# NTT123/vietTTS

Hardware: NVIDIA H100
Metric: audio_samples_per_sec (higher is better)
Workload: dtype f32 (bf16x3 split products on wgmma tensor cores, fp32 accumulate/storage)

## Files before the change

viettts_b200/csrc/tc_common.cuh:

```cuda
#pragma once
#include <cuda_bf16.h>
#include <stdint.h>

namespace tcx {

constexpr long long SPIN_TIMEOUT = 4000000000LL;

__device__ __forceinline__ uint32_t smem_u32(const void* p) { return (uint32_t)__cvta_generic_to_shared(p); }

__device__ __forceinline__ void mbar_init(uint64_t* bar, uint32_t count) {
  asm volatile("mbarrier.init.shared::cta.b64 [%0], %1;" ::"r"(smem_u32(bar)), "r"(count));
}
__device__ __forceinline__ void mbar_arrive(uint64_t* bar) {
  asm volatile("mbarrier.arrive.shared::cta.b64 _, [%0];" ::"r"(smem_u32(bar)) : "memory");
}
__device__ __forceinline__ void mbar_expect_tx(uint64_t* bar, uint32_t bytes) {
  asm volatile("mbarrier.arrive.expect_tx.shared::cta.b64 _, [%0], %1;" ::"r"(smem_u32(bar)), "r"(bytes) : "memory");
}
__device__ __forceinline__ bool mbar_try_wait(uint64_t* bar, uint32_t parity) {
  uint32_t ok;
  asm volatile(
      "{\n\t.reg .pred p;\n\t"
      "mbarrier.try_wait.parity.shared::cta.b64 p, [%1], %2;\n\t"
      "selp.u32 %0, 1, 0, p;\n\t}"
// ... 44 lines not shown
  if constexpr (F16) TCX_WGMMA_N32("f16"); else TCX_WGMMA_N32("bf16");
}
#define TCX_WGMMA_N64(TY)  \
  asm volatile(  \
      "{\n\t.reg .pred p;\n\t"  \
      "setp.ne.b32 p, %34, 0;\n\t"  \
      "wgmma.mma_async.sync.aligned.m64n64k16.f32." TY "." TY " "  \
      "{%0, %1, %2, %3, %4, %5, %6, %7, %8, %9, %10, %11, %12, %13, %14, %15, %16, %17, %18, %19, %20, %21, %22, %23, %24, %25, %26, %27, %28, %29, %30, %31}, "  \
      "%32, %33, p, 1, 1, 0, 0;\n\t}"  \
      : "+f"(d[0]), "+f"(d[1]), "+f"(d[2]), "+f"(d[3]), "+f"(d[4]), "+f"(d[5]), "+f"(d[6]), "+f"(d[7]), "+f"(d[8]), "+f"(d[9]), "+f"(d[10]), "+f"(d[11]), "+f"(d[12]), "+f"(d[13]), "+f"(d[14]), "+f"(d[15]), "+f"(d[16]), "+f"(d[17]), "+f"(d[18]), "+f"(d[19]), "+f"(d[20]), "+f"(d[21]), "+f"(d[22]), "+f"(d[23]), "+f"(d[24]), "+f"(d[25]), "+f"(d[26]), "+f"(d[27]), "+f"(d[28]), "+f"(d[29]), "+f"(d[30]), "+f"(d[31])  \
      : "l"(adesc), "l"(bdesc), "r"(accumulate)  \
  )
template <bool F16>
__device__ __forceinline__ void wgmma_n64(float (&d)[32], uint64_t adesc, uint64_t bdesc, uint32_t accumulate) {
  if constexpr (F16) TCX_WGMMA_N64("f16"); else TCX_WGMMA_N64("bf16");
}
#define TCX_WGMMA_N128(TY)  \
  asm volatile(  \
      "{\n\t.reg .pred p;\n\t"  \
      "setp.ne.b32 p, %66, 0;\n\t"  \
      "wgmma.mma_async.sync.aligned.m64n128k16.f32." TY "." TY " "  \
      "{%0, %1, %2, %3, %4, %5, %6, %7, %8, %9, %10, %11, %12, %13, %14, %15, %16, %17, %18, %19, %20, %21, %22, %23, %24, %25, %26, %27, %28, %29, %30, %31, %32, %33, %34, %35, %36, %37, %38, %39, %40, %41, %42, %43, %44, %45, %46, %47, %48, %49, %50, %51, %52, %53, %54, %55, %56, %57, %58, %59, %60, %61, %62, %63}, "  \
      "%64, %65, p, 1, 1, 0, 0;\n\t}"  \
      : "+f"(d[0]), "+f"(d[1]), "+f"(d[2]), "+f"(d[3]), "+f"(d[4]), "+f"(d[5]), "+f"(d[6]), "+f"(d[7]), "+f"(d[8]), "+f"(d[9]), "+f"(d[10]), "+f"(d[11]), "+f"(d[12]), "+f"(d[13]), "+f"(d[14]), "+f"(d[15]), "+f"(d[16]), "+f"(d[17]), "+f"(d[18]), "+f"(d[19]), "+f"(d[20]), "+f"(d[21]), "+f"(d[22]), "+f"(d[23]), "+f"(d[24]), "+f"(d[25]), "+f"(d[26]), "+f"(d[27]), "+f"(d[28]), "+f"(d[29]), "+f"(d[30]), "+f"(d[31]), "+f"(d[32]), "+f"(d[33]), "+f"(d[34]), "+f"(d[35]), "+f"(d[36]), "+f"(d[37]), "+f"(d[38]), "+f"(d[39]), "+f"(d[40]), "+f"(d[41]), "+f"(d[42]), "+f"(d[43]), "+f"(d[44]), "+f"(d[45]), "+f"(d[46]), "+f"(d[47]), "+f"(d[48]), "+f"(d[49]), "+f"(d[50]), "+f"(d[51]), "+f"(d[52]), "+f"(d[53]), "+f"(d[54]), "+f"(d[55]), "+f"(d[56]), "+f"(d[57]), "+f"(d[58]), "+f"(d[59]), "+f"(d[60]), "+f"(d[61]), "+f"(d[62]), "+f"(d[63])  \
      : "l"(adesc), "l"(bdesc), "r"(accumulate)  \
  )
template <bool F16>
__device__ __forceinline__ void wgmma_n128(float (&d)[64], uint64_t adesc, uint64_t bdesc, uint32_t accumulate) {
  if constexpr (F16) TCX_WGMMA_N128("f16"); else TCX_WGMMA_N128("bf16");
}
#define TCX_WGMMA_N256(TY)  \
  asm volatile(  \
      "{\n\t.reg .pred p;\n\t"  \
      "setp.ne.b32 p, %130, 0;\n\t"  \
      "wgmma.mma_async.sync.aligned.m64n256k16.f32." TY "." TY " "  \
      "{%0, %1, %2, %3, %4, %5, %6, %7, %8, %9, %10, %11, %12, %13, %14, %15, %16, %17, %18, %19, %20, %21, %22, %23, %24, %25, %26, %27, %28, %29, %30, %31, %32, %33, %34, %35, %36, %37, %38, %39, %40, %41, %42, %43, %44, %45, %46, %47, %48, %49, %50, %51, %52, %53, %54, %55, %56, %57, %58, %59, %60, %61, %62, %63, %64, %65, %66, %67, %68, %69, %70, %71, %72, %73, %74, %75, %76, %77, %78, %79, %80, %81, %82, %83, %84, %85, %86, %87, %88, %89, %90, %91, %92, %93, %94, %95, %96, %97, %98, %99, %100, %101, %102, %103, %104, %105, %106, %107, %108, %109, %110, %111, %112, %113, %114, %115, %116, %117, %118, %119, %120, %121, %122, %123, %124, %125, %126, %127}, "  \
      "%128, %129, p, 1, 1, 0, 0;\n\t}"  \
      : "+f"(d[0]), "+f"(d[1]), "+f"(d[2]), "+f"(d[3]), "+f"(d[4]), "+f"(d[5]), "+f"(d[6]), "+f"(d[7]), "+f"(d[8]), "+f"(d[9]), "+f"(d[10]), "+f"(d[11]), "+f"(d[12]), "+f"(d[13]), "+f"(d[14]), "+f"(d[15]), "+f"(d[16]), "+f"(d[17]), "+f"(d[18]), "+f"(d[19]), "+f"(d[20]), "+f"(d[21]), "+f"(d[22]), "+f"(d[23]), "+f"(d[24]), "+f"(d[25]), "+f"(d[26]), "+f"(d[27]), "+f"(d[28]), "+f"(d[29]), "+f"(d[30]), "+f"(d[31]), "+f"(d[32]), "+f"(d[33]), "+f"(d[34]), "+f"(d[35]), "+f"(d[36]), "+f"(d[37]), "+f"(d[38]), "+f"(d[39]), "+f"(d[40]), "+f"(d[41]), "+f"(d[42]), "+f"(d[43]), "+f"(d[44]), "+f"(d[45]), "+f"(d[46]), "+f"(d[47]), "+f"(d[48]), "+f"(d[49]), "+f"(d[50]), "+f"(d[51]), "+f"(d[52]), "+f"(d[53]), "+f"(d[54]), "+f"(d[55]), "+f"(d[56]), "+f"(d[57]), "+f"(d[58]), "+f"(d[59]), "+f"(d[60]), "+f"(d[61]), "+f"(d[62]), "+f"(d[63]), "+f"(d[64]), "+f"(d[65]), "+f"(d[66]), "+f"(d[67]), "+f"(d[68]), "+f"(d[69]), "+f"(d[70]), "+f"(d[71]), "+f"(d[72]), "+f"(d[73]), "+f"(d[74]), "+f"(d[75]), "+f"(d[76]), "+f"(d[77]), "+f"(d[78]), "+f"(d[79]), "+f"(d[80]), "+f"(d[81]), "+f"(d[82]), "+f"(d[83]), "+f"(d[84]), "+f"(d[85]), "+f"(d[86]), "+f"(d[87]), "+f"(d[88]), "+f"(d[89]), "+f"(d[90]), "+f"(d[91]), "+f"(d[92]), "+f"(d[93]), "+f"(d[94]), "+f"(d[95]), "+f"(d[96]), "+f"(d[97]), "+f"(d[98]), "+f"(d[99]), "+f"(d[100]), "+f"(d[101]), "+f"(d[102]), "+f"(d[103]), "+f"(d[104]), "+f"(d[105]), "+f"(d[106]), "+f"(d[107]), "+f"(d[108]), "+f"(d[109]), "+f"(d[110]), "+f"(d[111]), "+f"(d[112]), "+f"(d[113]), "+f"(d[114]), "+f"(d[115]), "+f"(d[116]), "+f"(d[117]), "+f"(d[118]), "+f"(d[119]), "+f"(d[120]), "+f"(d[121]), "+f"(d[122]), "+f"(d[123]), "+f"(d[124]), "+f"(d[125]), "+f"(d[126]), "+f"(d[127])  \
      : "l"(adesc), "l"(bdesc), "r"(accumulate)  \
  )
template <bool F16>
__device__ __forceinline__ void wgmma_n256(float (&d)[128], uint64_t adesc, uint64_t bdesc, uint32_t accumulate) {
  if constexpr (F16) TCX_WGMMA_N256("f16"); else TCX_WGMMA_N256("bf16");
}

template <int N, bool F16 = false>
__device__ __forceinline__ void wgmma(float (&d)[N / 2], uint64_t adesc, uint64_t bdesc, uint32_t accumulate) {
  if constexpr (N == 32) wgmma_n32<F16>(d, adesc, bdesc, accumulate);
  else if constexpr (N == 64) wgmma_n64<F16>(d, adesc, bdesc, accumulate);
  else if constexpr (N == 128) wgmma_n128<F16>(d, adesc, bdesc, accumulate);
  else wgmma_n256<F16>(d, adesc, bdesc, accumulate);
}

__device__ __forceinline__ void wgmma_rs_n32(float (&d)[16], const uint32_t (&a)[4], uint64_t bdesc, uint32_t accumulate) {
  asm volatile(
      "{\n\t.reg .pred p;\n\t"
      "setp.ne.b32 p, %21, 0;\n\t"
      "wgmma.mma_async.sync.aligned.m64n32k16.f32.bf16.bf16 "
      "{%0, %1, %2, %3, %4, %5, %6, %7, %8, %9, %10, %11, %12, %13, %14, %15}, "
      "{%16, %17, %18, %19}, %20, p, 1, 1, 0;\n\t}"
      : "+f"(d[0]), "+f"(d[1]), "+f"(d[2]), "+f"(d[3]), "+f"(d[4]), "+f"(d[5]), "+f"(d[6]), "+f"(d[7]), "+f"(d[8]), "+f"(d[9]), "+f"(d[10]), "+f"(d[11]), "+f"(d[12]), "+f"(d[13]), "+f"(d[14]), "+f"(d[15])
      : "r"(a[0]), "r"(a[1]), "r"(a[2]), "r"(a[3]), "l"(bdesc), "r"(accumulate));
}
__device__ __forceinline__ void wgmma_rs_n64(float (&d)[32], const uint32_t (&a)[4], uint64_t bdesc, uint32_t accumulate) {
  asm volatile(
      "{\n\t.reg .pred p;\n\t"
      "setp.ne.b32 p, %37, 0;\n\t"
      "wgmma.mma_async.sync.aligned.m64n64k16.f32.bf16.bf16 "
      "{%0, %1, %2, %3, %4, %5, %6, %7, %8, %9, %10, %11, %12, %13, %14, %15, %16, %17, %18, %19, %20, %21, %22, %23, %24, %25, %26, %27, %28, %29, %30, %31}, "
      "{%32, %33, %34, %35}, %36, p, 1, 1, 0;\n\t}"
      : "+f"(d[0]), "+f"(d[1]), "+f"(d[2]), "+f"(d[3]), "+f"(d[4]), "+f"(d[5]), "+f"(d[6]), "+f"(d[7]), "+f"(d[8]), "+f"(d[9]), "+f"(d[10]), "+f"(d[11]), "+f"(d[12]), "+f"(d[13]), "+f"(d[14]), "+f"(d[15]), "+f"(d[16]), "+f"(d[17]), "+f"(d[18]), "+f"(d[19]), "+f"(d[20]), "+f"(d[21]), "+f"(d[22]), "+f"(d[23]), "+f"(d[24]), "+f"(d[25]), "+f"(d[26]), "+f"(d[27]), "+f"(d[28]), "+f"(d[29]), "+f"(d[30]), "+f"(d[31])
      : "r"(a[0]), "r"(a[1]), "r"(a[2]), "r"(a[3]), "l"(bdesc), "r"(accumulate));
}

template <int N>
__device__ __forceinline__ void wgmma_rs(float (&d)[N / 2], const uint32_t (&a)[4], uint64_t bdesc, uint32_t accumulate) {
  if constexpr (N == 32) wgmma_rs_n32(d, a, bdesc, accumulate);
  else wgmma_rs_n64(d, a, bdesc, accumulate);
}
__device__ __forceinline__ void ldmatrix_x4(uint32_t (&r)[4], uint32_t saddr) {
  asm volatile("ldmatrix.sync.aligned.m8n8.x4.shared.b16 {%0, %1, %2, %3}, [%4];"
               : "=r"(r[0]), "=r"(r[1]), "=r"(r[2]), "=r"(r[3]) : "r"(saddr) : "memory");
}

__device__ __forceinline__ void named_bar(int id, int nthreads) { asm volatile("bar.sync %0, %1;" ::"r"(id), "r"(nthreads) : "memory"); }

__device__ __forceinline__ float4 ldg_pf256(const float* p) {
  float4 v;
  asm volatile("ld.global.nc.L2::256B.v4.f32 {%0, %1, %2, %3}, [%4];" : "=f"(v.x), "=f"(v.y), "=f"(v.z), "=f"(v.w) : "l"(p));
  return v;
}

__device__ __forceinline__ float lrelu(float v, float s) { return fmaxf(v, s * v); }

__device__ __forceinline__ void split4(const float4 v, uint2& hi, uint2& lo) {
  const __nv_bfloat162 h01 = __floats2bfloat162_rn(v.x, v.y);
  const __nv_bfloat162 h23 = __floats2bfloat162_rn(v.z, v.w);
  const uint32_t u01 = *reinterpret_cast<const uint32_t*>(&h01);
  const uint32_t u23 = *reinterpret_cast<const uint32_t*>(&h23);
  const float r0 = v.x - __uint_as_float(u01 << 16);
  const float r1 = v.y - __uint_as_float(u01 & 0xffff0000u);
  const float r2 = v.z - __uint_as_float(u23 << 16);
  const float r3 = v.w - __uint_as_float(u23 & 0xffff0000u);
  const __nv_bfloat162 l01 = __floats2bfloat162_rn(r0, r1);
  const __nv_bfloat162 l23 = __floats2bfloat162_rn(r2, r3);
  hi.x = u01;
  hi.y = u23;
  lo.x = *reinterpret_cast<const uint32_t*>(&l01);
  lo.y = *reinterpret_cast<const uint32_t*>(&l23);
}

__device__ __forceinline__ uint32_t f16x2_sat(float v0, float v1) {
  uint32_t r;
  asm("cvt.rn.satfinite.f16x2.f32 %0, %1, %2;" : "=r"(r) : "f"(v1), "f"(v0));
  return r;
}
__device__ __forceinline__ uint2 f16x4_sat(const float4 v) { return make_uint2(f16x2_sat(v.x, v.y), f16x2_sat(v.z, v.w)); }

}
```

viettts_b200/csrc/tc_conv.cu:

```cuda
#include <cuda_bf16.h>

#include <algorithm>

#include "tc_common.cuh"
#include "vtts_internal.cuh"

namespace {

using namespace tcx;

constexpr int NCWG = 2;
constexpr int NCONS = NCWG * 128;
constexpr int PROD_WARP = NCONS / 32;
constexpr int NCONV = 96;
constexpr int NTHREADS = NCONS + 32 + NCONV;
constexpr int NA = 4;
constexpr int HALO = 64;
constexpr int PAIR_OVERLAP = 16;
constexpr int NQ = 2;
constexpr int NREADERS = (NCONS + NCONV) / 32;

constexpr int SUB_CG = 4;
constexpr int SUB_HALO = 1;
constexpr int SUB_RS = NCWG * 64 + SUB_HALO;
// ... 218 lines not shown
          wgmma_rs<N>(acc[mt], fa_hi[mt], b_lo, 1u);
          wgmma_rs<N>(acc[mt], fa_lo[mt], b_hi, 1u);
        }
        wgmma_commit();
        wgmma_wait<0>();
        if (lane == 0) mbar_arrive(&w_empty[rw.s]);
        rw.next<NW>();
        continue;
      }
      wgmma_fence();
#pragma unroll
      for (int mt = 0; mt < MW; ++mt) {
        const uint32_t row = a_base + ((wg * MW + mt) * 64 + j * dil) * 16;
        const uint64_t a_hi = a_tmpl | (uint64_t)(row >> 4);
        const uint64_t a_lo = a_tmpl | (uint64_t)((row + 2 * RA * 16) >> 4);
        if constexpr (F16) {
          wgmma<N, true>(acc[mt], a_hi, b_hi, first);
        } else {
          wgmma<N>(acc[mt], a_hi, b_hi, first);
          wgmma<N>(acc[mt], a_hi, b_lo, 1u);
          wgmma<N>(acc[mt], a_lo, b_hi, 1u);
        }
      }
      wgmma_commit();
      wgmma_wait<1>();
      if (lane0) {
        if (pend_w >= 0) mbar_arrive(&w_empty[pend_w]);
        if (pend_a >= 0) mbar_arrive(&a_empty[pend_a]);
      }
      pend_w = (int)rw.s;
      pend_a = (A_FROM_RING && j == k - 1) ? (int)ra.s : -1;
      rw.next<NW>();
    }
    if constexpr (A_FROM_RING) ra.next<NA>();
  }
  wgmma_wait<0>();
  if (lane0) {
    if (pend_w >= 0) mbar_arrive(&w_empty[pend_w]);
    if (pend_a >= 0) mbar_arrive(&a_empty[pend_a]);
  }
}

template <int N, int NW, int NAS, bool F16>
__device__ __forceinline__ void consume_rows(float (&acc)[N / 2], int wg, uint32_t a_st_u32, uint64_t* a_full, uint64_t* a_empty, Ring& ra,
                                             uint32_t w_st_u32, uint64_t* w_full, uint64_t* w_empty, Ring& rw, int nch, int k, int dil,
                                             int* err, long long& w_a, long long& w_w) {
  const uint64_t a_tmpl = make_desc(0, SUB_RS * 16, 128);
  const uint64_t b_tmpl = make_desc(0, (F16 ? 1 : 2) * N * 16, 128);
  const bool lane0 = (threadIdx.x & 31) == 0;
  int pend_w = -1, pend_a = -1;
  for (int c0 = 0; c0 < nch; c0 += SUB_CG) {
    mbar_wait_t(&a_full[ra.s], ra.p, err, 2, w_a);
    const uint32_t a_blk = a_st_u32 + ra.s * SUB_STAGE + wg * 64 * 16;
    for (int cl = 0; cl < SUB_CG; ++cl) {
      for (int j = 0; j < k; ++j) {
        mbar_wait_t(&w_full[rw.s], rw.p, err, 3, w_w);
        const uint32_t w_base = w_st_u32 + rw.s * (N * 64);
        const uint64_t b_hi = b_tmpl | (uint64_t)(w_base >> 4);
        const uint64_t b_lo = b_tmpl | (uint64_t)((w_base + N * 16) >> 4);
        const uint32_t first = ((c0 + cl) | j) != 0 ? 1u : 0u;
        const uint32_t row = a_blk + cl * SUB_CSB + j * dil * 16;
        const uint64_t a_hi = a_tmpl | (uint64_t)(row >> 4);
        const uint64_t a_lo = a_tmpl | (uint64_t)((row + 2 * SUB_RS * 16) >> 4);
        wgmma_fence();
        if constexpr (F16) {
          wgmma<N, true>(acc, a_hi, b_hi, first);
        } else {
          wgmma<N>(acc, a_hi, b_hi, first);
          wgmma<N>(acc, a_hi, b_lo, 1u);
          wgmma<N>(acc, a_lo, b_hi, 1u);
        }
        wgmma_commit();
        wgmma_wait<1>();
        if (lane0) {
          if (pend_w >= 0) mbar_arrive(&w_empty[pend_w]);
          if (pend_a >= 0) mbar_arrive(&a_empty[pend_a]);
        }
        pend_w = (int)rw.s;
        pend_a = (cl == SUB_CG - 1 && j == k - 1) ? (int)ra.s : -1;
        rw.next<NW>();
      }
    }
    ra.next<NAS>();
  }
  wgmma_wait<0>();
  if (lane0) {
    if (pend_w >= 0) mbar_arrive(&w_empty[pend_w]);
    if (pend_a >= 0) mbar_arrive(&a_empty[pend_a]);
  }
}

__device__ __forceinline__ void cp_async16(void* smem_dst, const void* gsrc) {
  asm volatile("cp.async.cg.shared.global [%0], [%1], 16;" ::"r"(smem_u32(smem_dst)), "l"(gsrc) : "memory");
}
__device__ __forceinline__ void cp_async_commit() { asm volatile("cp.async.commit_group;" ::: "memory"); }
__device__ __forceinline__ void cp_async_wait_all() { asm volatile("cp.async.wait_all;" ::: "memory"); }

__device__ __forceinline__ void init_barriers(uint64_t* bars, int nw) {
  uint64_t* a_full = bars;
  uint64_t* a_empty = bars + NA;
  uint64_t* w_full = bars + 2 * NA;
  uint64_t* w_empty = bars + 2 * NA + nw;
  uint64_t* q_full = bars + 2 * NA + 2 * nw;
  uint64_t* q_empty = q_full + NQ;
  for (int i = 0; i < NA; ++i) { mbar_init(&a_full[i], NCONV); mbar_init(&a_empty[i], NCONS / 32); }
  for (int i = 0; i < nw; ++i) { mbar_init(&w_full[i], 1); mbar_init(&w_empty[i], NCONS / 32); }
  for (int i = 0; i < NQ; ++i) { mbar_init(&q_full[i], 1); mbar_init(&q_empty[i], NREADERS); }
  asm volatile("fence.mbarrier_init.release.cluster;" ::: "memory");
}

__device__ __forceinline__ TileQueue tile_queue(uint64_t* bars, int nw) {
  uint64_t* q_full = bars + 2 * NA + 2 * nw;
  return TileQueue{reinterpret_cast<int*>(q_full + 2 * NQ), q_full, q_full + NQ, Ring{}};
}

__device__ __forceinline__ int sub_elem(const TcLaunch& L, const TcProb& P, int tau, int col) {
  return (tau * P.out_stride + P.out_off) * L.out_ld + P.out_e0 + col;
}

#define PRODUCER_TILES                                                                     \
  TileQueue q = tile_queue(bars, NW);                                                      \
  long long w_q = 0;                                                                       \
  int t_next = blockIdx.x;                                                                 \
  q.put(t_next, L.err, w_q);                                                               \
  auto next_tile = [&]() {                                                                 \
    const int t = t_next;                                                                  \
    if (t >= 0) { t_next = take_ticket(L.sched, L.ntiles); q.put(t_next, L.err, w_q); }    \
    return t;                                                                              \
  };
#define READER_TILES                                                                       \
  TileQueue q = tile_queue(bars, NW);                                                      \
  long long w_q = 0;                                                                       \
  auto next_tile = [&]() { return q.get(L.err, w_q); };

template <int N, int EPI, int MW, bool F16, bool SUB>
__global__ void __launch_bounds__(NTHREADS, 1) tc_conv_kernel(const __grid_constant__ TcLaunch L) {
  static_assert(!SUB || EPI == 0, "sub-row output uses the plain epilogue");
  using Cfg = TcCfg<N, MW, 0, EPI == 0, SUB>;
  constexpr int R = Cfg::R, RA = Cfg::RA, NW = Cfg::NW, NAS = Cfg::NAS;
  extern __shared__ uint8_t smem_raw[];
  uint8_t* smem = (uint8_t*)(((uintptr_t)smem_raw + 1023) & ~(uintptr_t)1023);
  uint8_t* a_st = smem;
  uint8_t* w_st = smem + Cfg::A_BYTES;
  float* epi_st = reinterpret_cast<float*>(smem_raw + (w_st + NW * Cfg::W_STAGE - smem_raw));
  uint64_t* bars = reinterpret_cast<uint64_t*>(w_st + NW * Cfg::W_STAGE + Cfg::EPI_STAGE);
  uint64_t* a_full = bars;
  uint64_t* a_empty = bars + NA;
  uint64_t* w_full = bars + 2 * NA;
  uint64_t* w_empty = bars + 2 * NA + NW;

  const int tid = threadIdx.x;
  const int warp = __shfl_sync(0xffffffffu, tid >> 5, 0);
  if (tid == 0) init_barriers(bars, NW);
  __syncthreads();

  const int nch = L.Cin / 16;

  constexpr bool ROW_BOUNDS = EPI == 0;
#define TILE_LOOP_BEGIN                                                           \
  for (int tile; (tile = next_tile()) >= 0;) {                                    \
    const Tile td = decode_tile(tile, L.nprob, L.tiles_per_row);                   \
    const int b = td.b;                                                            \
    const int tau0 = td.tt * R;                                                    \
    const TcProb& P = L.p[td.pi];                                                  \
    int valid = L.T_rows, in_lo = 0, out_hi = 0;                                  \
    if (ROW_BOUNDS && P.rb) {                                                     \
// ... 110 lines not shown
#pragma unroll
        for (int mt = 0; mt < MW; ++mt) {
          const int blk = blk_row(mt);
          if (SUB ? sub_elem(L, P, blk, 0) >= e_lim : !row_ok(blk)) break;
#pragma unroll
          for (int nh = 0; nh < N / EPI_NC; ++nh) {
            if (mt + nh > 0 && P.resid) {
              fetch_pass(mt, nh);
              wait_pass();
            }
#pragma unroll
            for (int jn = 0; jn < EPI_NC / 8; ++jn) {
              const int col = jn * 8 + fc, e = (nh * (EPI_NC / 8) + jn) * 4;
              const float2 bi = *reinterpret_cast<const float2*>(stg_bias + nh * EPI_NC + col);
#pragma unroll
              for (int h = 0; h < 2; ++h) {
                float2* s = reinterpret_cast<float2*>(stg + (fr + 8 * h) * EPI_LD + col);
                float2 o = make_float2(acc[mt][e + 2 * h] + bi.x, acc[mt][e + 2 * h + 1] + bi.y);
                if (P.resid) {
                  const float2 r = *s;
                  o.x += r.x; o.y += r.y;
                }
                *s = o;
              }
            }
            named_bar(2 + wg, 128);
#pragma unroll
            for (int i = 0; i < NQ4; ++i) {
              const int row = i * RPS + dr, tau = blk + row;
              const int e = (tau * ostride + ooff) * L.out_ld + oe0 + nh * EPI_NC + dq * 4;
              if (elem_ok(tau, e))
                *reinterpret_cast<float4*>(P.out + out_base + e) = *reinterpret_cast<const float4*>(stg + row * EPI_LD + dq * 4);
            }
            named_bar(2 + wg, 128);
          }
        }
      } else {
        const int row_w = tau0 + wg * MW * 64 + (warp & 3) * 16 + (lane >> 2);
#pragma unroll
        for (int mt = 0; mt < MW; ++mt)
#pragma unroll
          for (int h = 0; h < 2; ++h) {
            const int tau = row_w + mt * 64 + 8 * h;
            if (!row_ok(tau)) continue;
            const size_t orow = out_base + (size_t)(tau * ostride + ooff) * L.out_ld;
#pragma unroll
            for (int jn = 0; jn < N / 8; ++jn) {
              const int col = jn * 8 + 2 * (lane & 3);
              if (col >= n_valid) continue;
              float2 o = make_float2(acc[mt][jn * 4 + 2 * h], acc[mt][jn * 4 + 2 * h + 1]);
              const float2 bi = __ldg(reinterpret_cast<const float2*>(P.bias + col));
              o.x += bi.x; o.y += bi.y;
              if (P.bn_mean) {
                const float2 mu = __ldg(reinterpret_cast<const float2*>(P.bn_mean + col));
                const float2 iv = __ldg(reinterpret_cast<const float2*>(P.bn_inv + col));
                const float2 of = __ldg(reinterpret_cast<const float2*>(P.bn_off + col));
                o.x = (o.x - mu.x) * iv.x + of.x; o.y = (o.y - mu.y) * iv.y + of.y;
              }
              if (post_act == 1) { o.x = tanhf(o.x); o.y = tanhf(o.y); }
              else if (post_act == 2) { o.x = fmaxf(o.x, 0.f); o.y = fmaxf(o.y, 0.f); }
              if (P.resid) {
                const float2 r = __ldg(reinterpret_cast<const float2*>(P.resid + orow + col));
                o.x += r.x; o.y += r.y;
              }
              *reinterpret_cast<float2*>(P.out + orow + col) = o;
            }
          }
      }
      t_epi += clock64() - t_epi0;
    TILE_LOOP_END
    if (L.dbg && tid == 0) {
      long long* d = L.dbg + (size_t)blockIdx.x * 16;
      d[0] = clock64() - t_begin; d[1] = t_epi; d[2] = w_a; d[3] = w_w;
    }
  }
#undef TILE_LOOP_BEGIN
#undef TILE_LOOP_END
}

template <int N, int MW, bool A2_REGS, bool F16>
__global__ void __launch_bounds__(NTHREADS, 1) tc_pair_kernel(const __grid_constant__ TcPairLaunch L) {
  using Cfg = TcCfg<N, MW, 1>;
  constexpr int R = Cfg::R, R_OUT = Cfg::R_OUT, RA = Cfg::RA, NW = Cfg::NW, NCH = N / 16;
  extern __shared__ uint8_t smem_raw[];
  uint8_t* smem = (uint8_t*)(((uintptr_t)smem_raw + 1023) & ~(uintptr_t)1023);
  uint8_t* a_st = smem;
  uint8_t* w_st = smem + NA * Cfg::A_STAGE;
  uint8_t* mid = w_st + NW * Cfg::W_STAGE;
  uint64_t* bars = reinterpret_cast<uint64_t*>(mid + Cfg::NCH2 * Cfg::A_STAGE);
  uint64_t* a_full = bars;
  uint64_t* a_empty = bars + NA;
  uint64_t* w_full = bars + 2 * NA;
  uint64_t* w_empty = bars + 2 * NA + NW;

  const int tid = threadIdx.x;
  const int warp = __shfl_sync(0xffffffffu, tid >> 5, 0);
  if (tid == 0) init_barriers(bars, NW);
  __syncthreads();

#define TILE_LOOP_BEGIN                                                   \
  for (int tile; (tile = next_tile()) >= 0;) {                            \
    const Tile td = decode_tile(tile, L.nprob, L.tiles_per_row);        \
    const int b = td.b;                                                    \
    const int tau0 = td.tt * R_OUT;                                        \
    int valid = L.T_rows;                                                 \
    if (L.len) {                                                          \
      const int v = L.len[b] * L.len_mul;                                 \
      valid = v < valid ? v : valid;                                      \
    }                                                                     \
    if (tau0 >= valid) continue;                                          \
    const TcPairProb& P = L.p[td.pi];                                      \
    const int k = P.k, dil = P.dil, h2 = (k - 1) / 2;
#define TILE_LOOP_END }

  if (warp == PROD_WARP) {
    if ((tid & 31) == 0) {
      Ring rw;
      long long w_e = 0;
      PRODUCER_TILES
      TILE_LOOP_BEGIN
        (void)b; (void)tau0; (void)dil; (void)h2;
        produce_weights<N, NW, F16>(w_st, w_full, w_empty, rw, P.w1pk, NCH, k, L.err, w_e);
        produce_weights<N, NW, F16>(w_st, w_full, w_empty, rw, P.w2pk, NCH, k, L.err, w_e);
      TILE_LOOP_END
    }
  } else if (warp > PROD_WARP) {
    const int ct = tid - NCONS - 32;
    Ring ra;
    long long w_ae = 0;
    READER_TILES
    TILE_LOOP_BEGIN
      const float* x = P.x + (size_t)b * L.T_rows * N;
      const int row_base = tau0 - h2 - (k - 1) * dil / 2;
      for (int c = 0; c < NCH; ++c) {
        mbar_wait_t(&a_empty[ra.s], ra.p ^ 1, L.err, 5, w_ae);
        convert_chunk<RA, F16>(a_st + ra.s * Cfg::A_STAGE, ct, x, nullptr, nullptr, N, c, row_base, R + (k - 1) * dil, 0, valid, 1, L.slope);
        fence_proxy_async();
        mbar_arrive(&a_full[ra.s]);
        ra.next<NA>();
      }
    TILE_LOOP_END
  } else {
    const int wg = warp >> 2, lane = tid & 31;
    float acc[MW][N / 2];
    Ring ra, rw;
    long long w_a = 0, w_w = 0;
    const long long t_begin = clock64();
    const float slope = L.slope;
    READER_TILES
    TILE_LOOP_BEGIN
      consume<N, MW, RA, NW, true, false, F16>(acc, wg, smem_u32(a_st), a_full, a_empty, ra, smem_u32(w_st), w_full, w_empty, rw, NCH, k, dil,
                                               L.err, w_a, w_w);
      const int lr_w = wg * MW * 64 + (warp & 3) * 16 + (lane >> 2);
#pragma unroll
      for (int mt = 0; mt < MW; ++mt)
#pragma unroll
        for (int h = 0; h < 2; ++h) {
          const int lr = lr_w + mt * 64 + 8 * h;
          const int u = tau0 - h2 + lr;
          const bool inside = u >= 0 && u < valid;
#pragma unroll
          for (int jn = 0; jn < N / 8; ++jn) {
            const int col = jn * 8 + 2 * (lane & 3);
            const float2 bi = __ldg(reinterpret_cast<const float2*>(P.b1 + col));
            const float v0 = inside ? lrelu(acc[mt][jn * 4 + 2 * h] + bi.x, slope) : 0.f;
            const float v1 = inside ? lrelu(acc[mt][jn * 4 + 2 * h + 1] + bi.y, slope) : 0.f;
            uint8_t* dst = mid + (col >> 4) * Cfg::A_STAGE + (((col >> 3) & 1) * RA + lr) * 16 + (col & 7) * 2;
            if constexpr (F16) {
              *reinterpret_cast<uint32_t*>(dst) = f16x2_sat(v0, v1);
            } else {
              const __nv_bfloat162 hi = __floats2bfloat162_rn(v0, v1);
              const __nv_bfloat162 lo = __floats2bfloat162_rn(v0 - __low2float(hi), v1 - __high2float(hi));
              *reinterpret_cast<__nv_bfloat162*>(dst) = hi;
              *reinterpret_cast<__nv_bfloat162*>(dst + 2 * RA * 16) = lo;
            }
          }
        }
      fence_proxy_async();
      named_bar(1, NCONS);
      consume<N, MW, RA, NW, false, A2_REGS, F16>(acc, wg, smem_u32(mid), a_full, a_empty, ra, smem_u32(w_st), w_full, w_empty, rw, NCH, k, 1,
                                                  L.err, w_a, w_w);
      named_bar(1, NCONS);
      const float* x = P.x + (size_t)b * L.T_rows * N;
      float* out = P.out + (size_t)b * L.T_rows * N;
#pragma unroll
      for (int mt = 0; mt < MW; ++mt)
#pragma unroll
        for (int h = 0; h < 2; ++h) {
          const int lr = lr_w + mt * 64 + 8 * h;
          const int tau = tau0 + lr;
          if (lr >= R_OUT || tau >= valid) continue;
#pragma unroll
          for (int jn = 0; jn < N / 8; ++jn) {
            const int col = jn * 8 + 2 * (lane & 3);
            const float2 bi = __ldg(reinterpret_cast<const float2*>(P.b2 + col));
            const float2 r = __ldg(reinterpret_cast<const float2*>(x + (size_t)tau * N + col));
            float2 o;
            o.x = acc[mt][jn * 4 + 2 * h] + bi.x + r.x;
            o.y = acc[mt][jn * 4 + 2 * h + 1] + bi.y + r.y;
            *reinterpret_cast<float2*>(out + (size_t)tau * N + col) = o;
          }
        }
    TILE_LOOP_END
    if (L.dbg && tid == 0) {
      long long* d = L.dbg + (size_t)blockIdx.x * 16;
      d[0] = clock64() - t_begin; d[2] = w_a; d[3] = w_w;
    }
  }
#undef TILE_LOOP_BEGIN
#undef TILE_LOOP_END
}

template <bool F16>
__global__ void pack_w_kernel(const float* __restrict__ w, uint16_t* __restrict__ dst, int k, int Cin, int Cout_total, int n0, int N) {
  const size_t total = (size_t)k * Cin * N;
  for (size_t idx = blockIdx.x * (size_t)blockDim.x + threadIdx.x; idx < total; idx += (size_t)gridDim.x * blockDim.x) {
    const int n = idx % N;
    const int i = (idx / N) % Cin;
    const int j = idx / ((size_t)N * Cin);
    const float v = (n0 + n) < Cout_total ? w[((size_t)j * Cin + i) * Cout_total + n0 + n] : 0.f;
    const int c = i / 16, kh = (i % 16) / 8, e = i % 8;
    if constexpr (F16) {
      const size_t blk = ((size_t)c * k + j) * (size_t)(2 * N * 8);
      dst[blk + ((size_t)kh * N + n) * 8 + e] = (uint16_t)(f16x2_sat(v, 0.f) & 0xffffu);
// ... 100 lines not shown
    cursor += (vtts_tc_packed_elems(k, Cin, N, f16) * 2 + 255) & ~size_t(255);
  }
  return VTTS_OK;
}

int vtts_conv_dispatch(vtts_ctx* ctx, const ConvLaunch& L, void* const* wpk, cudaStream_t st) {
  if (ctx->precision == VTTS_PRECISION_FP32 || wpk == nullptr) return vtts_launch_conv(ctx, L, st);
  const int N = vtts_tc_tile_n(L.Cout), nt = (L.Cout + N - 1) / N;
  TcLaunch TL;
  auto reset = [&]() {
    memset(&TL, 0, sizeof(TL));
    TL.Cin = L.Cin; TL.N = N; TL.in_ld = L.Cin; TL.out_ld = L.Cout; TL.B = L.B; TL.T_rows = L.T_rows; TL.rows_out = L.rows_out;
    TL.len = L.len; TL.len_mul = L.len_mul; TL.pre_mode = L.pre_mode; TL.pre_slope = L.pre_slope; TL.post_act = L.post_act;
    TL.n_valid = (L.Cout % N) ? (L.Cout % N) : N;
  };
  reset();
  for (int pass = 0; pass < 2; ++pass) {
    const bool partial = pass == 1;
    if (partial && (L.Cout % N) == 0) break;
    reset();
    TL.n_valid = partial ? (L.Cout % N) : N;
    for (int pi = 0; pi < L.nprob; ++pi) {
      const ConvProb& cp = L.p[pi];
      for (int t = 0; t < nt; ++t) {
        const bool is_partial = (t == nt - 1) && (L.Cout % N) != 0;
        if (is_partial != partial) continue;
        const int n0 = t * N;
        TcProb q;
        memset(&q, 0, sizeof(q));
        q.x0 = cp.x0; q.x1 = cp.x1; q.x2 = cp.x2;
        q.wpk = wpk[pi * nt + t];
        q.bias = cp.bias + n0;
        q.resid = cp.resid ? cp.resid + n0 : nullptr;
        if (cp.bn_mean) { q.bn_mean = cp.bn_mean + n0; q.bn_inv = cp.bn_inv + n0; q.bn_off = cp.bn_off + n0; }
        q.out = cp.out + n0;
        q.k = cp.k; q.dil = cp.dil; q.in_off = cp.in_off; q.out_stride = cp.out_stride; q.out_off = cp.out_off;
        TL.p[TL.nprob++] = q;
        if (TL.nprob == 8) {
          int rc = vtts_launch_tc_conv(ctx, TL, st);
          if (rc) return rc;
          TL.nprob = 0;
        }
      }
    }
    if (TL.nprob > 0) {
      int rc = vtts_launch_tc_conv(ctx, TL, st);
      if (rc) return rc;
    }
  }
  return VTTS_OK;
}

int vtts_launch_tc_conv(vtts_ctx* ctx, TcLaunch& L, cudaStream_t st) {
  if (L.nprob < 1 || L.nprob > 8) return ctx->fail(VTTS_ERR_BAD_ARG, "tc_conv: nprob %d", L.nprob);
  if (L.Cin % 16 != 0) return ctx->fail(VTTS_ERR_BAD_ARG, "tc_conv: Cin %d", L.Cin);
  for (int i = 0; i < L.nprob; ++i)
    if (L.p[i].k < 1) return ctx->fail(VTTS_ERR_BAD_ARG, "tc_conv: k");
  L.sched = ctx->d_tc_sched;
  L.err = ctx->d_err;
  L.dbg = ctx->tc_dbg_on ? ctx->d_tc_dbg : nullptr;
  switch (L.N) {
    case 256: return launch_n<256>(ctx, L, st);
    case 128: return launch_n<128>(ctx, L, st);
    case 64: return launch_n<64>(ctx, L, st);
    case 32: return launch_n<32>(ctx, L, st);
    default: return ctx->fail(VTTS_ERR_BAD_ARG, "tc_conv: N %d unsupported", L.N);
  }
}

int vtts_launch_tc_pair(vtts_ctx* ctx, TcPairLaunch& L, cudaStream_t st) {
  if (L.nprob < 1 || L.nprob > 3) return ctx->fail(VTTS_ERR_BAD_ARG, "tc_pair: nprob %d", L.nprob);
  for (int i = 0; i < L.nprob; ++i)
    if (L.p[i].k < 1 || L.p[i].x == L.p[i].out) return ctx->fail(VTTS_ERR_BAD_ARG, "tc_pair: bad problem %d", i);
  L.sched = ctx->d_tc_sched;
  L.err = ctx->d_err;
  L.dbg = ctx->tc_dbg_on ? ctx->d_tc_dbg : nullptr;
  if (L.N != 32 && L.N != 64) return ctx->fail(VTTS_ERR_BAD_ARG, "tc_pair: C %d unsupported (32 or 64)", L.N);
  if (L.f16) {
    if (ctx->pair_ts != 2) return ctx->fail(VTTS_ERR_BAD_ARG, "tc_pair: fp16 operands exist for the default pair form (256-row tiles) only, not form %d", ctx->pair_ts);
    return L.N == 64 ? launch_pair<64, 2, false, true>(ctx, L, st) : launch_pair<32, 2, false, true>(ctx, L, st);
  }
  if (ctx->pair_ts == 1) return L.N == 64 ? launch_pair<64, 2, true>(ctx, L, st) : launch_pair<32, 2, true>(ctx, L, st);
  if (ctx->pair_ts == 0) return L.N == 64 ? launch_pair<64, 1, false>(ctx, L, st) : launch_pair<32, 1, false>(ctx, L, st);
  return L.N == 64 ? launch_pair<64, 2, false>(ctx, L, st) : launch_pair<32, 2, false>(ctx, L, st);
}
```

Before: 58.24 million.

## Use channel-major wgmma path with stmatrix transpose for 64-channel pair conv

Adds a channel-major consumer path for the default 64-channel, 256-row pair kernel. Weights become the M operand and time rows the N=128 operand. The intermediate activation is split into bf16 hi/lo and written with stmatrix.trans, replacing the per-element store path. The output epilogue stages accumulators in shared memory so that residual add and global stores use coalesced float4 accesses. This restructures data reuse and the epilogue cost, but it adds extra named barriers and an alignment requirement on x and out.

```diff
diff --git a/viettts_b200/csrc/tc_common.cuh b/viettts_b200/csrc/tc_common.cuh
--- a/viettts_b200/csrc/tc_common.cuh
+++ b/viettts_b200/csrc/tc_common.cuh
@@ -150,6 +150,11 @@
   asm volatile("ldmatrix.sync.aligned.m8n8.x4.shared.b16 {%0, %1, %2, %3}, [%4];"
                : "=r"(r[0]), "=r"(r[1]), "=r"(r[2]), "=r"(r[3]) : "r"(saddr) : "memory");
 }
+__device__ __forceinline__ void stmatrix_x4_trans(uint32_t saddr, const uint32_t (&r)[4]) {
+  asm volatile("stmatrix.sync.aligned.m8n8.x4.trans.shared.b16 [%0], {%1, %2, %3, %4};" ::"r"(saddr), "r"(r[0]), "r"(r[1]), "r"(r[2]),
+               "r"(r[3])
+               : "memory");
+}
 
 __device__ __forceinline__ void named_bar(int id, int nthreads) { asm volatile("bar.sync %0, %1;" ::"r"(id), "r"(nthreads) : "memory"); }
 
diff --git a/viettts_b200/csrc/tc_conv.cu b/viettts_b200/csrc/tc_conv.cu
--- a/viettts_b200/csrc/tc_conv.cu
+++ b/viettts_b200/csrc/tc_conv.cu
@@ -324,6 +324,54 @@
       }
     }
     ra.next<NAS>();
+  }
+  wgmma_wait<0>();
+  if (lane0) {
+    if (pend_w >= 0) mbar_arrive(&w_empty[pend_w]);
+    if (pend_a >= 0) mbar_arrive(&a_empty[pend_a]);
+  }
+}
+
+template <int RA, int NW, bool A_FROM_RING>
+__device__ __forceinline__ void consume_cm(float (&acc)[64], int wg, uint32_t x_st_u32, uint64_t* a_full, uint64_t* a_empty, Ring& ra,
+                                           uint32_t w_st_u32, uint64_t* w_full, uint64_t* w_empty, Ring& rw, int nch, int k, int dil,
+                                           int* err, long long& w_a, long long& w_w) {
+  constexpr int N = 64;
+  const uint64_t x_tmpl = make_desc(0, RA * 16, 128);
+  const uint64_t w_tmpl = make_desc(0, 2 * N * 16, 128);
+  const bool lane0 = (threadIdx.x & 31) == 0;
+  int pend_w = -1, pend_a = -1;
+  for (int c = 0; c < nch; ++c) {
+    uint32_t x_base;
+    if constexpr (A_FROM_RING) {
+      mbar_wait_t(&a_full[ra.s], ra.p, err, 2, w_a);
+      x_base = x_st_u32 + ra.s * (RA * 64);
+    } else {
+      x_base = x_st_u32 + c * (RA * 64);
+    }
+    for (int j = 0; j < k; ++j) {
+      mbar_wait_t(&w_full[rw.s], rw.p, err, 3, w_w);
+      const uint32_t w_base = w_st_u32 + rw.s * (N * 64);
+      const uint32_t row = x_base + (wg * 128 + j * dil) * 16;
+      const uint64_t x_hi = x_tmpl | (uint64_t)(row >> 4);
+      const uint64_t x_lo = x_tmpl | (uint64_t)((row + 2 * RA * 16) >> 4);
+      const uint64_t w_hi = w_tmpl | (uint64_t)(w_base >> 4);
+      const uint32_t first = (c | j) != 0 ? 1u : 0u;
+      wgmma_fence();
+      wgmma<128>(acc, w_hi, x_hi, first);
+      wgmma<128>(acc, w_tmpl | (uint64_t)((w_base + N * 16) >> 4), x_hi, 1u);
+      wgmma<128>(acc, w_hi, x_lo, 1u);
+      wgmma_commit();
+      wgmma_wait<1>();
+      if (lane0) {
+        if (pend_w >= 0) mbar_arrive(&w_empty[pend_w]);
+        if (pend_a >= 0) mbar_arrive(&a_empty[pend_a]);
+      }
+      pend_w = (int)rw.s;
+      pend_a = (A_FROM_RING && j == k - 1) ? (int)ra.s : -1;
+      rw.next<NW>();
+    }
+    if constexpr (A_FROM_RING) ra.next<NA>();
   }
   wgmma_wait<0>();
   if (lane0) {
@@ -600,6 +648,7 @@
 __global__ void __launch_bounds__(NTHREADS, 1) tc_pair_kernel(const __grid_constant__ TcPairLaunch L) {
   using Cfg = TcCfg<N, MW, 1>;
   constexpr int R = Cfg::R, R_OUT = Cfg::R_OUT, RA = Cfg::RA, NW = Cfg::NW, NCH = N / 16;
+  constexpr bool CM = N == 64 && MW == 2 && !A2_REGS && !F16;
   extern __shared__ uint8_t smem_raw[];
   uint8_t* smem = (uint8_t*)(((uintptr_t)smem_raw + 1023) & ~(uintptr_t)1023);
   uint8_t* a_st = smem;
@@ -658,6 +707,82 @@
         ra.next<NA>();
       }
     TILE_LOOP_END
+  } else if constexpr (CM) {
+    const int wg = warp >> 2, lane = tid & 31, w4 = warp & 3, g = lane >> 2, tq = lane & 3;
+    float acc[64];
+    Ring ra, rw;
+    long long w_a = 0, w_w = 0;
+    const long long t_begin = clock64();
+    const float slope = L.slope;
+    auto vt = [&](int i) { return 8 * (i >> 2) + 2 * tq + (i & 1); };
+    auto vco = [&](int i) { return 16 * w4 + g + 8 * ((i >> 1) & 1); };
+    const int mi = lane >> 3, rr = lane & 7;
+    const uint32_t st_lane = smem_u32(mid) + w4 * Cfg::A_STAGE + (mi & 1) * RA * 16 + (wg * 128 + 8 * (mi >> 1) + rr) * 16;
+    constexpr int EPI_LD = N + 4, Q4 = N / 4, RPP = 128 / Q4, NPASS = 128 / RPP;
+    static_assert(NCWG * 128 * EPI_LD * 4 <= Cfg::NCH2 * Cfg::A_STAGE, "staging fits in the intermediate");
+    float* stg = reinterpret_cast<float*>(smem_raw + (mid - smem_raw)) + wg * 128 * EPI_LD;
+    const int rq = (tid & 127) % Q4, r0 = (tid & 127) / Q4;
+    READER_TILES
+    TILE_LOOP_BEGIN
+      consume_cm<RA, NW, true>(acc, wg, smem_u32(a_st), a_full, a_empty, ra, smem_u32(w_st), w_full, w_empty, rw, NCH, k, dil, L.err, w_a,
+                                  w_w);
+      named_bar(1, NCONS);
+      {
+        const float b1a = __ldg(P.b1 + vco(0)), b1b = __ldg(P.b1 + vco(2));
+#pragma unroll
+        for (int p = 0; p < 8; ++p) {
+          uint32_t rh[4], rl[4];
+#pragma unroll
+          for (int m = 0; m < 4; ++m) {
+            float y[2];
+#pragma unroll
+            for (int e = 0; e < 2; ++e) {
+              const int i = 8 * p + 2 * m + e;
+              const int u = tau0 - h2 + wg * 128 + vt(i);
+              y[e] = u >= 0 && u < valid ? lrelu(acc[i] + (i & 2 ? b1b : b1a), slope) : 0.f;
+            }
+            const __nv_bfloat162 hi = __floats2bfloat162_rn(y[0], y[1]);
+            const __nv_bfloat162 lo = __floats2bfloat162_rn(y[0] - __low2float(hi), y[1] - __high2float(hi));
+            rh[m] = *reinterpret_cast<const uint32_t*>(&hi);
+            rl[m] = *reinterpret_cast<const uint32_t*>(&lo);
+          }
+          stmatrix_x4_trans(st_lane + p * 256, rh);
+          stmatrix_x4_trans(st_lane + p * 256 + 2 * RA * 16, rl);
+        }
+      }
+      fence_proxy_async();
+      named_bar(1, NCONS);
+      consume_cm<RA, NW, false>(acc, wg, smem_u32(mid), a_full, a_empty, ra, smem_u32(w_st), w_full, w_empty, rw, NCH, k, 1, L.err, w_a,
+                                   w_w);
+      named_bar(1, NCONS);
+      const float* x = P.x + (size_t)b * L.T_rows * N;
+      float* out = P.out + (size_t)b * L.T_rows * N;
+      float4 res[NPASS];
+#pragma unroll
+      for (int s = 0; s < NPASS; ++s) {
+        const int lr = wg * 128 + r0 + s * RPP, tau = tau0 + lr;
+        res[s] = make_float4(0.f, 0.f, 0.f, 0.f);
+        if (lr < R_OUT && tau < valid) res[s] = __ldg(reinterpret_cast<const float4*>(x + (size_t)tau * N + rq * 4));
+      }
+      {
+        const float b2a = __ldg(P.b2 + vco(0)), b2b = __ldg(P.b2 + vco(2));
+#pragma unroll
+        for (int i = 0; i < 64; ++i) stg[vt(i) * EPI_LD + vco(i)] = acc[i] + (i & 2 ? b2b : b2a);
+      }
+      named_bar(2 + wg, 128);
+#pragma unroll
+      for (int s = 0; s < NPASS; ++s) {
+        const int lr = wg * 128 + r0 + s * RPP, tau = tau0 + lr;
+        if (lr >= R_OUT || tau >= valid) continue;
+        const float4 a = *reinterpret_cast<const float4*>(stg + (r0 + s * RPP) * EPI_LD + rq * 4);
+        *reinterpret_cast<float4*>(out + (size_t)tau * N + rq * 4) =
+            make_float4(a.x + res[s].x, a.y + res[s].y, a.z + res[s].z, a.w + res[s].w);
+      }
+    TILE_LOOP_END
+    if (L.dbg && tid == 0) {
+      long long* d = L.dbg + (size_t)blockIdx.x * 16;
+      d[0] = clock64() - t_begin; d[2] = w_a; d[3] = w_w;
+    }
   } else {
     const int wg = warp >> 2, lane = tid & 31;
     float acc[MW][N / 2];
@@ -924,5 +1049,7 @@
   }
   if (ctx->pair_ts == 1) return L.N == 64 ? launch_pair<64, 2, true>(ctx, L, st) : launch_pair<32, 2, true>(ctx, L, st);
   if (ctx->pair_ts == 0) return L.N == 64 ? launch_pair<64, 1, false>(ctx, L, st) : launch_pair<32, 1, false>(ctx, L, st);
+  for (int i = 0; i < L.nprob && L.N == 64; ++i)
+    if ((((uintptr_t)L.p[i].x | (uintptr_t)L.p[i].out) & 15) != 0) return ctx->fail(VTTS_ERR_BAD_ARG, "tc_pair: x and out must be 16-byte aligned");
   return L.N == 64 ? launch_pair<64, 2, false>(ctx, L, st) : launch_pair<32, 2, false>(ctx, L, st);
 }
```

Result: no change. 58.82 million, median of 6 (+1.0%).
